# acids-ircam/RAVE

Hardware: NVIDIA H100
Metric: audio-seconds/s (v2 train step fwd+bwd, 48 kHz) (higher is better)
Workload: dtype bf16

## Files before the change

include/rave_b200.h:

```cpp
#ifndef RAVE_B200_H
#define RAVE_B200_H

#include <stddef.h>
#include <stdint.h>

#ifdef __cplusplus
extern "C" {
#endif

#define RAVE_ACT_NONE 0
#define RAVE_ACT_LEAKY 1
#define RAVE_ACT_SNAKE 2

#define RAVE_PREC_FP32 0
#define RAVE_PREC_BF16 1
#define RAVE_PREC_TF32 2

int rave_b200_version(void);
const char *rave_b200_last_error(void);
unsigned long long rave_b200_launch_count(void);

int rave_pqmf_analysis_fwd(const float *x, const float *taps, float *y, int B, int T, int Lout,
                           int ntaps, int pad_l, int flip_sign, void *stream);
int rave_pqmf_synthesis_fwd(const float *x, const float *w, float *out, int B, int L, int K,
// ... 9 lines not shown
                           const float *alpha, int post_act, float post_slope, const float *post_x,
                           const float *post_alpha, void *stream);
int rave_conv1d_scatter_f32(const float *src, const float *w, const float *bias, const float *res,
                            float *out, int B, int Cs, int Ls, int Cm, int Lo, int K, int stride,
                            int dil, int pad_l, long ws_m, long ws_c, int act, float slope,
                            const float *alpha, int post_act, float post_slope, const float *post_x,
                            const float *post_alpha, void *stream);

size_t rave_conv1d_wgrad_workspace_bytes(int B, int Ca, int Cc, int Lp, int K);
int rave_conv1d_wgrad_f32(const float *P, const float *Q, float *dw, int B, int Ca, int Lp, int Cc,
                          int Lq, int K, int stride, int dil, int pad_l, long os_a, long os_c,
                          int act_p, int act_q, float slope, const float *alpha, void *workspace,
                          void *stream);

int rave_weight_norm_fwd(const float *v, const float *g, float *w, float *norm_out, int C0, int R,
                         void *stream);
int rave_weight_norm_bwd(const float *dw, const float *v, const float *g, const float *norm,
                         float *dv, float *dg, int C0, int R, void *stream);

int rave_act_fwd(const float *x, float *y, int B, int C, int L, int act, float slope,
                 const float *alpha, void *stream);
int rave_act_bwd(const float *dy, const float *x, float *dx, float *dalpha, int B, int C, int L,
                 int act, float slope, const float *alpha, void *stream);
int rave_am_tanh_fwd(const float *x, float *y, int B, int C, int L, void *stream);
int rave_am_tanh_bwd(const float *dy, const float *x, float *dx, int B, int C, int L, void *stream);
int rave_reparam_fwd(const float *z, const float *eps, float *zs, float *kl_sum, int B, int C, int L, void *stream);

int rave_conv1d_tc_supported(int Cin, int Cout, int K, int stride, int dil);
int rave_dilated_unit_tc_supported(int C, int L);
int rave_dilated_unit_tc_fwd(const void *xa_bf16, const void *w3t_bf16, const void *w1t_bf16, void *a1_out,
                             float *out_f32, void *out_act, int B, int C, int L, int pitch, int dil, int pad_l,
                             float slope_in, float slope_mid, int act_out, float slope_out, void *stream);
int rave_conv1d_tc_plan(int B, int Cin, int Cout, int Lout, int K);
int rave_conv1d_tc_fwd(const void *xa_bf16, const void *wt_bf16, const float *bias, const float *res,
                       const void *res_bf16, const void *dact_src_bf16, const void *res_act_bf16, float res_slope,
                       float *out_f32, void *out_act_bf16,
                       int B, int Cin, int Lin, int in_pitch, int Cout, int Lout,
                       int K, int stride, int dil, int pad_l, int act, float slope, int out_rows,
                       int out_row_stride, int out_row_offset, const float *fm_d, int fm_bh, void *stream);
int rave_conv1d_tc_fwd_x3(const void *xa_bf16, const void *wt_bf16, const float *bias, const float *res,
                          const void *res_act, float res_slope, float *out_f32, void *out_act, int B, int Cin, int Lin,
                          int in_pitch, int Cout, int Lout, int K, int stride, int dil, int pad_l, int act, float slope,
                          int out_rows, int out_row_stride, int out_row_offset, int act_cs, void *stream);
int rave_conv1d_tc_wgrad_splits(int B, int Cm, int Lp, int Cn, int K);
int rave_time_stack_cl(const float *x, void *out_bf16, int B, int C, int T, int F, int Fp, int Cp, int kt, int pt,
                       void *stream);
int rave_time_stack_cl_bwd(const void *g_bf16, float *gx, int B, int C, int T, int F, int Fp, int Cp, int kt, int pt,
                           void *stream);
int rave_time_stack_nhwc(const float *x, void *out_bf16, int B, int C, int T, int F, long sb, long st, int Fp, int Cp, int kt,
                         int pt, void *stream);
int rave_time_stack_nhwc_bwd(const void *g_bf16, float *gx, int B, int C, int T, int F, int Fp, int Cp, int kt, int pt,
                             void *stream);
int rave_time_stack_nhwc_dil(const float *x, void *out_bf16, int B, int C, int T, int F, long sb, long st, int Fp, int Cp,
                             int kt, int pt, int dil, void *stream);
int rave_time_stack_nhwc_dil_bwd(const void *g_bf16, float *gx, int B, int C, int T, int F, int Fp, int Cp, int kt, int pt,
                                 int dil, void *stream);
int rave_l1_stats_f32(const float *t, const float *v, float *stats, long n, void *stream);
int rave_l1_grad_f32(const float *t, const float *v, const float *d, float *gt, float *gv, long n, void *stream);
int rave_leaky_fm_fwd(const float *x, float *a, float *stats, long H, float slope, void *stream);
int rave_leaky_fm_bwd(const float *a, const float *g, const float *d, float *gx, long H, float slope, void *stream);
int rave_leaky_fm_stack_fwd(const float *x, float *a, float *stats, void *xs_bf16, long Rh, int T, int F, int C, int Fp,
                            float slope, void *stream);
int rave_leaky_fm_stack_bwd(const float *a, const void *gxs_bf16, const float *ga, const float *d, float *gx, long Rh, int T,
                            int F, int C, int Fp, float slope, void *stream);
int rave_leaky_fm_stack_dil_fwd(const float *x, float *a, float *stats, void *xs_bf16, long Rh, int T, int F, int C, int Fp,
                                int dil, float slope, void *stream);
// ... 99 lines not shown
```

rave_b200/_lib.py:

```python
import ctypes
import os
from ctypes import c_float, c_int, c_long, c_size_t, c_ulonglong, c_void_p, c_char_p

_HERE = os.path.dirname(os.path.abspath(__file__))
LIB_PATH = os.path.join(_HERE, "csrc", "librave_b200.so")

_P, _I, _F, _L = c_void_p, c_int, c_float, c_long

SIGNATURES = {
    "rave_b200_version": (c_int, []),
    "rave_b200_last_error": (c_char_p, []),
    "rave_b200_launch_count": (c_ulonglong, []),
    "rave_pqmf_analysis_fwd": (c_int, [_P, _P, _P, _I, _I, _I, _I, _I, _I, _P]),
    "rave_pqmf_synthesis_fwd": (c_int, [_P, _P, _P, _I, _I, _I, _I, _F, _I, _P]),
    "rave_pqmf_analysis_fast": (c_int, [_P, _P, _P, _P, _I, _I, _I, _I, _I, _P]),
    "rave_pqmf_synthesis_fast": (c_int, [_P, _P, _P, _P, _I, _I, _I, _F, _I, _P]),
    "rave_conv1d_gather_f32": (c_int, [_P, _P, _P, _P, _P, _I, _I, _I, _I, _I, _I, _I, _I, _I, _L, _L,
                                       _I, _F, _P, _I, _F, _P, _P, _P]),
    "rave_conv1d_scatter_f32": (c_int, [_P, _P, _P, _P, _P, _I, _I, _I, _I, _I, _I, _I, _I, _I, _L, _L,
                                        _I, _F, _P, _I, _F, _P, _P, _P]),
    "rave_conv1d_wgrad_workspace_bytes": (c_size_t, [_I, _I, _I, _I, _I]),
    "rave_conv1d_wgrad_f32": (c_int, [_P, _P, _P, _I, _I, _I, _I, _I, _I, _I, _I, _I, _L, _L, _I, _I,
                                      _F, _P, _P, _P]),
    "rave_weight_norm_fwd": (c_int, [_P, _P, _P, _P, _I, _I, _P]),
    "rave_weight_norm_bwd": (c_int, [_P, _P, _P, _P, _P, _P, _I, _I, _P]),
    "rave_act_fwd": (c_int, [_P, _P, _I, _I, _I, _I, _F, _P, _P]),
    "rave_act_bwd": (c_int, [_P, _P, _P, _P, _I, _I, _I, _I, _F, _P, _P]),
    "rave_am_tanh_fwd": (c_int, [_P, _P, _I, _I, _I, _P]),
    "rave_am_tanh_bwd": (c_int, [_P, _P, _P, _I, _I, _I, _P]),
    "rave_reparam_fwd": (c_int, [_P, _P, _P, _P, _I, _I, _I, _P]),
    "rave_conv1d_tc_supported": (c_int, [_I, _I, _I, _I, _I]),
    "rave_dilated_unit_tc_supported": (c_int, [_I, _I]),
    "rave_dilated_unit_tc_fwd": (c_int, [_P, _P, _P, _P, _P, _P, _I, _I, _I, _I, _I, _I, _F, _F, _I, _F, _P]),
    "rave_conv1d_tc_plan": (c_int, [_I, _I, _I, _I, _I]),
    "rave_conv1d_tc_fwd": (c_int, [_P, _P, _P, _P, _P, _P, _P, _F, _P, _P, _I, _I, _I, _I, _I, _I, _I, _I, _I, _I, _I,
                                   _F, _I, _I, _I, _P, _I, _P]),
    "rave_conv1d_tc_fwd_x3": (c_int, [_P, _P, _P, _P, _P, _F, _P, _P, _I, _I, _I, _I, _I, _I, _I, _I, _I, _I, _I, _F, _I,
                                      _I, _I, _I, _P]),
    "rave_weight_prep_tc_multi_x3": (c_int, [_I, _P, _P]),
    "rave_ncl_to_cl_x3": (c_int, [_P, _P, _I, _I, _I, _P]),
    "rave_conv1d_tc_wgrad": (c_int, [_P, _P, _P, _P, _I, _I, _I, _I, _I, _I, _I, _I, _I, _I, _I, _P]),
    "rave_tapmajor_to_weight_f32": (c_int, [_P, _P, _I, _I, _I, _I, _I, _P]),
    "rave_conv1d_tc_wgrad_splits": (c_int, [_I, _I, _I, _I, _I]),
    "rave_time_stack_cl": (c_int, [_P, _P, _I, _I, _I, _I, _I, _I, _I, _I, _P]),
    "rave_time_stack_cl_bwd": (c_int, [_P, _P, _I, _I, _I, _I, _I, _I, _I, _I, _P]),
    "rave_time_stack_nhwc": (c_int, [_P, _P, _I, _I, _I, _I, ctypes.c_long, ctypes.c_long, _I, _I, _I, _I, _P]),
    "rave_time_stack_nhwc_bwd": (c_int, [_P, _P, _I, _I, _I, _I, _I, _I, _I, _I, _P]),
    "rave_time_stack_nhwc_dil": (c_int, [_P, _P, _I, _I, _I, _I, ctypes.c_long, ctypes.c_long, _I, _I, _I, _I, _I, _P]),
    "rave_time_stack_nhwc_dil_bwd": (c_int, [_P, _P, _I, _I, _I, _I, _I, _I, _I, _I, _I, _P]),
    "rave_l1_stats_f32": (c_int, [_P, _P, _P, ctypes.c_long, _P]),
    "rave_leaky_fm_fwd": (c_int, [_P, _P, _P, ctypes.c_long, ctypes.c_float, _P]),
    "rave_leaky_fm_bwd": (c_int, [_P, _P, _P, _P, ctypes.c_long, ctypes.c_float, _P]),
    "rave_leaky_fm_stack_fwd": (c_int, [_P, _P, _P, _P, ctypes.c_long, _I, _I, _I, _I, ctypes.c_float, _P]),
    "rave_leaky_fm_stack_bwd": (c_int, [_P, _P, _P, _P, _P, ctypes.c_long, _I, _I, _I, _I, ctypes.c_float, _P]),
    "rave_leaky_fm_stack_dil_fwd": (c_int, [_P, _P, _P, _P, ctypes.c_long, _I, _I, _I, _I, _I, ctypes.c_float, _P]),
    "rave_leaky_fm_stack_dil_bwd": (c_int, [_P, _P, _P, _P, _P, ctypes.c_long, _I, _I, _I, _I, _I, ctypes.c_float, _P]),
    "rave_l1_grad_f32": (c_int, [_P, _P, _P, _P, _P, ctypes.c_long, _P]),
    "rave_snake_cl_fwd": (c_int, [_P, _P, _P, ctypes.c_long, _I, _P]),
    "rave_snake_cl_bwd": (c_int, [_P, _P, _P, _P, _P, _P, ctypes.c_long, _I, _P]),
    "rave_weight_prep_tc": (c_int, [_P, _P, _P, _P, _P, _I, _P, _P, _I, _I, _I, _I, _I, _I, _P]),
    "rave_weight_norm_bwd_tapmajor": (c_int, [_P, _P, _P, _P, _P, _P, _I, _I, _I, _I, _I, _I, _P]),
    "rave_conv1d_c1_fwd": (c_int, [_P, _P, _P, _P, _P, _I, _I, _I, _I, _I, _I, _I, _I, _I, _I, _F, _P]),
    "rave_conv1d_c1_wgrad_splits": (c_int, [_I, _I]),
    "rave_conv1d_c1_wgrad": (c_int, [_P, _P, _P, _I, _I, _I, _I, _I, _I, _I, _I, _I, _I, _P]),
    "rave_conv1d_c1_dgrad": (c_int, [_P, _P, _P, _I, _I, _I, _I, _I, _I, _I, _I, _I, _I, _P]),
    "rave_colsum_bf16": (c_int, [_P, _P, _I, _I, _I, _I, _I, _P]),
    "rave_im2col_c1": (c_int, [_P, _P, _I, _I, _I, _I, _I, _I, _I, _I, _I, _I, _I, _P]),
# ... 109 lines not shown
```

rave_b200/csrc/conv_tc.cu:

```cuda
#include <string.h>

#include "common.cuh"
#include "tc_common.cuh"

namespace rave {
namespace tc {

constexpr int BLOCK_M = 128;
constexpr int NUM_THREADS = 288;
constexpr int SMEM_MAX = 227 * 1024;

struct TcParams {
  int B, Cin, Lin, Cout, Lout, K, stride, dil, pad_l;
  int BL, BB;
  int n_lt, n_bg, n_nt;
  int num_kb;
  int act;
  float slope;
  const float *bias;
  const float *res;
  const __nv_bfloat16 *res_bf16;
  const __nv_bfloat16 *dact_src;
  const __nv_bfloat16 *res_act;
  float res_inv_slope;
  float *out_f32;
  __nv_bfloat16 *out_act;
  int out_rows;
  int out_row_stride;
  int out_row_offset;
  const float *fm_d;
  long fm_half;
  int fm_bh;
  int x3;
  int act_ld;
  int act_cs;
  int stages, nacc;
  int stg;
  int acc_off, stg_off, bar_off;
};

template <int BLOCK_N, int BLOCK_K, bool X3 = false>
struct SmemLayout {
  static constexpr int PARTS = X3 ? 2 : 1;
  static constexpr int A_PART = BLOCK_M * BLOCK_K * 2;
  static constexpr int B_PART = (BLOCK_N * BLOCK_K * 2 + 1023) / 1024 * 1024;
  static constexpr int A_BYTES = PARTS * A_PART;
  static constexpr int B_BYTES = PARTS * BLOCK_N * BLOCK_K * 2;
  static constexpr int B_BYTES_PAD = PARTS * B_PART;
  static constexpr int STAGE_BYTES = A_BYTES + B_BYTES_PAD;
  static constexpr int ACC_LD = acc_pitch(BLOCK_N);
  static constexpr int ACC_BYTES = BLOCK_M * ACC_LD * 4;
  static constexpr int OUT_BOXC = BLOCK_N % 64 == 0 ? 64 : BLOCK_N % 32 == 0 ? 32 : 16;
  static constexpr int OUT_SPAN = OUT_BOXC * 2;
  static constexpr int STG_BYTES = X3 ? 0 : BLOCK_M * BLOCK_N * 2;
  static constexpr int FIXED = 256 + 1024;
  static constexpr int stages_for(int nacc, int stg) {
    const int s = (SMEM_MAX - FIXED - nacc * ACC_BYTES - stg * STG_BYTES) / STAGE_BYTES;
    return s > 8 ? 8 : s;
  }
};

template <int BLOCK_N, int BLOCK_K, bool X3>
static void plan_smem(int kblocks, TcParams &p) {
  using L = SmemLayout<BLOCK_N, BLOCK_K, X3>;
  const int base = L::stages_for(1, 0);
  const int need = kblocks + 1 < base ? kblocks + 1 : base;
  p.nacc = 1;
  p.stg = 0;
  if (L::stages_for(2, 1) >= need) { p.nacc = 2; p.stg = 1; }
  else if (L::stages_for(1, 1) >= need) p.stg = 1;
  if (X3) p.stg = 0;
// ... 289 lines not shown
      const int bg = mt / p.n_lt;
      const int n0 = nt * BLOCK_N;
      const int b = bg * p.BB + row / p.BL;
      const int l = lt * p.BL + row % p.BL;
      const bool valid = (b < p.B) && (l < p.Lout);
      const size_t orow = (size_t)b * p.out_rows + (size_t)l * p.out_row_stride + p.out_row_offset;

      const int buf = p.nacc == 2 ? (it & 1) : 0;
      const uint32_t use = p.nacc == 2 ? (it >> 1) : it;
      if (stg) {
        if (issuer) bulk_wait_read<0>();
        named_bar_sync(1, 128);
      }
      mbar_wait(&tfull_bar[buf], use & 1);
      const uint32_t taddr = (uint32_t)(128 * buf + quad * 32) << 16;
      tc_epilogue<BLOCK_N, X3, BOXC>(p, taddr, n0, valid, orow, p.fm_d ? (b < p.fm_bh ? 1 : -1) : 0, stg, row);
      __syncwarp();
      if (lane == 0) mbar_arrive(&tempty_bar[buf]);
      if (stg) {
        fence_proxy_async();
        named_bar_sync(1, 128);
        if (issuer) {
#pragma unroll
          for (int c = 0; c < BLOCK_N; c += BOXC)
            tma_store_3d(&tmap_o, stg + (c / BOXC) * (BLOCK_M * L::OUT_SPAN), n0 + c, lt * p.BL, bg * p.BB);
          bulk_commit();
        }
      }
    }
    if (stg && issuer) bulk_wait_all();
  }
}

typedef CUresult (*EncodeTiledFn)(CUtensorMap *, CUtensorMapDataType, cuuint32_t, void *, const cuuint64_t *,
                                  const cuuint64_t *, const cuuint32_t *, const cuuint32_t *,
                                  CUtensorMapInterleave, CUtensorMapSwizzle, CUtensorMapL2promotion,
                                  CUtensorMapFloatOOBfill);

static EncodeTiledFn get_encode_fn() {
  static EncodeTiledFn fn = nullptr;
  if (!fn) {
    void *ptr = nullptr;
    cudaDriverEntryPointQueryResult q;
    if (cudaGetDriverEntryPoint("cuTensorMapEncodeTiled", &ptr, cudaEnableDefault, &q) == cudaSuccess &&
        q == cudaDriverEntryPointSuccess)
      fn = (EncodeTiledFn)ptr;
  }
  return fn;
}

static CUtensorMapSwizzle swizzle_enum(int bytes) {
  return bytes == 128 ? CU_TENSOR_MAP_SWIZZLE_128B : bytes == 64 ? CU_TENSOR_MAP_SWIZZLE_64B
                                                                 : CU_TENSOR_MAP_SWIZZLE_32B;
}

static int pick_block_k(int Cin) {
  if (Cin % 64 == 0) return 64;
  if (Cin % 32 == 0) return 32;
  if (Cin % 16 == 0) return 16;
  return 0;
}

static int pick_block_n(int Cout, long m_tiles) {
  const int cands[] = {128, 96, 64, 48, 32, 16};
  constexpr int NC = sizeof(cands) / sizeof(cands[0]);
  int best = 0;
  for (int c : cands) {
    if (Cout % c) continue;
    if (!best) best = c;
    if (m_tiles * (Cout / c) >= 132) return c;
  }
  for (int i = NC - 1; i >= 0; --i)
    if (Cout % cands[i] == 0 && cands[i] >= 32) return cands[i];
  return best;
}

template <int BN, int BK, bool X3>
static int launch(const CUtensorMap &ta, const CUtensorMap &tb, TcParams p, cudaStream_t stream) {
  using L = SmemLayout<BN, BK, X3>;
  plan_smem<BN, BK, X3>(p.K * p.num_kb, p);
  if (!p.out_act) p.stg = 0;
  const int smem = p.bar_off + L::FIXED;
  static int attr = 0;
  if (smem > attr) {
    cudaError_t e = cudaFuncSetAttribute(conv_tc_kernel<BN, BK, X3>, cudaFuncAttributeMaxDynamicSharedMemorySize, smem);
    if (e != cudaSuccess) {
      set_error("conv1d_tc: cudaFuncSetAttribute(%d bytes): %s", smem, cudaGetErrorString(e));
      return 2;
    }
    attr = smem;
  }
  CUtensorMap to;
  memset(&to, 0, sizeof(to));
  if (p.stg) {
    EncodeTiledFn enc = get_encode_fn();
    cuuint64_t dims[3] = {(cuuint64_t)p.Cout, (cuuint64_t)p.Lout, (cuuint64_t)p.B};
    cuuint64_t strides[2] = {(cuuint64_t)p.Cout * 2 * p.out_row_stride, (cuuint64_t)p.Cout * 2 * p.out_rows};
    cuuint32_t box[3] = {(cuuint32_t)L::OUT_BOXC, (cuuint32_t)p.BL, (cuuint32_t)p.BB};
    cuuint32_t estr[3] = {1, 1, 1};
    CUresult r = enc(&to, CU_TENSOR_MAP_DATA_TYPE_BFLOAT16, 3, p.out_act + (size_t)p.out_row_offset * p.Cout, dims,
                     strides, box, estr, CU_TENSOR_MAP_INTERLEAVE_NONE, swizzle_enum(L::OUT_SPAN),
                     CU_TENSOR_MAP_L2_PROMOTION_NONE, CU_TENSOR_MAP_FLOAT_OOB_FILL_NONE);
    if (r != CUDA_SUCCESS) {
      set_error("conv1d_tc: output tensor map encode failed (%d)", (int)r);
      return 1;
    }
  }
  const int tiles = p.n_lt * p.n_bg * p.n_nt;
  int dev = 0, sms = 132;
  cudaGetDevice(&dev);
  cudaDeviceGetAttribute(&sms, cudaDevAttrMultiProcessorCount, dev);
  const int grid = tiles < sms ? tiles : sms;
  launch_pdl(conv_tc_kernel<BN, BK, X3>, dim3(grid), dim3(NUM_THREADS), smem, stream, ta, tb, to, p);
  RAVE_CHECK_LAUNCH("conv1d_tc");
  return 0;
}

template <int BK, bool X3>
static int dispatch_n(int bn, const CUtensorMap &ta, const CUtensorMap &tb, const TcParams &p,
                      cudaStream_t s) {
  switch (bn) {
    case 128: return launch<128, BK, X3>(ta, tb, p, s);
    case 96: return launch<96, BK, X3>(ta, tb, p, s);
    case 64: return launch<64, BK, X3>(ta, tb, p, s);
    case 48: return launch<48, BK, X3>(ta, tb, p, s);
    case 32: return launch<32, BK, X3>(ta, tb, p, s);
    case 16: return launch<16, BK, X3>(ta, tb, p, s);
  }
  set_error("conv1d_tc: no kernel for BLOCK_N=%d", bn);
  return 1;
}

template <int BK>
static int smem_plan_bits(int BN, int kblocks) {
  TcParams q;
  switch (BN) {
    case 128: plan_smem<128, BK, false>(kblocks, q); break;
    case 96: plan_smem<96, BK, false>(kblocks, q); break;
    case 64: plan_smem<64, BK, false>(kblocks, q); break;
    case 48: plan_smem<48, BK, false>(kblocks, q); break;
// ... 17 lines not shown

int conv_tc_dispatch_x3(int BK, int BN, const CUtensorMap &ta, const CUtensorMap &tb, const TcParams &p, cudaStream_t s);
#ifdef RAVE_TC_X3_UNIT
int conv_tc_dispatch_x3(int BK, int BN, const CUtensorMap &ta, const CUtensorMap &tb, const TcParams &p, cudaStream_t s) {
  return dispatch_all<true>(BK, BN, ta, tb, p, s);
}
#endif

}
}

#ifndef RAVE_TC_X3_UNIT
extern "C" int rave_conv1d_tc_supported(int Cin, int Cout, int K, int stride, int dil) {
  if (rave::tc::pick_block_k(Cin) == 0) return 0;
  if (Cout % 16) return 0;
  if (K < 1 || stride < 1 || dil < 1) return 0;
  return 1;
}

extern "C" int rave_conv1d_tc_plan(int B, int Cin, int Cout, int Lout, int K) {
  using namespace rave;
  using namespace rave::tc;
  const int BK = pick_block_k(Cin);
  if (!BK || Cout % 16) return 0;
  int BL = 128;
  while (BL > Lout && BL > 8) BL >>= 1;
  const long m_tiles = (long)ceil_div(Lout, BL) * ceil_div(B, 128 / BL);
  const int BN = pick_block_n(Cout, m_tiles);
  if (!BN) return 0;
  const int kblocks = K * ceil_div(Cin, BK);
  const int smem = BK == 64 ? smem_plan_bits<64>(BN, kblocks)
                 : BK == 32 ? smem_plan_bits<32>(BN, kblocks) : smem_plan_bits<16>(BN, kblocks);
  return BN | (BK << 12) | smem;
}

static int conv1d_tc_fwd_impl(const void *xa, const void *wt, const float *bias, const float *res,
                              const void *res_bf16, const void *dact_src, const void *res_act, float res_slope,
                              float *out_f32, void *out_act,
                              int B, int Cin, int Lin, int in_pitch, int Cout, int Lout,
                              int K, int stride, int dil, int pad_l, int act, float slope, int out_rows,
                              int out_row_stride, int out_row_offset, const float *fm_d, int fm_bh,
                              void *stream, int x3, int act_cs = 0) {
  using namespace rave;
  using namespace rave::tc;
  RAVE_CHECK_ARG(!x3 || (!res_bf16 && !dact_src && !fm_d),
                 "conv1d_tc(x3): the split-operand mode has no gradient epilogues (forward path only)");
  RAVE_CHECK_ARG(xa && wt && (out_f32 || out_act), "conv1d_tc: null pointer");
  RAVE_CHECK_ARG(rave_conv1d_tc_supported(Cin, Cout, K, stride, dil), "conv1d_tc: unsupported shape Cin=%d Cout=%d",
                 Cin, Cout);
  if (in_pitch <= 0) in_pitch = Lin;
  RAVE_CHECK_ARG(in_pitch >= ceil_div(Lin, stride) * stride,
                 "conv1d_tc: input pitch %d < Lin %d rounded up to the stride %d (slack rows must be zero)", in_pitch,
                 Lin, stride);
  RAVE_CHECK_ARG(act == RAVE_ACT_NONE || act == RAVE_ACT_LEAKY, "conv1d_tc: epilogue activation %d unsupported", act);
  RAVE_CHECK_ARG(act != RAVE_ACT_LEAKY || (slope >= 0.f && slope <= 1.f), "conv1d_tc: LeakyReLU slope %g outside [0, 1]",
                 (double)slope);
  RAVE_CHECK_ARG(!res_act || (res_slope > 0.f && res_slope <= 1.f), "conv1d_tc: res_slope %g outside (0, 1]",
                 (double)res_slope);
  RAVE_CHECK_ARG(((uintptr_t)bias & 15) == 0, "conv1d_tc: bias must be 16-byte aligned");
  RAVE_CHECK_ARG(((uintptr_t)xa & 15) == 0 && ((uintptr_t)wt & 15) == 0, "conv1d_tc: operands must be 16B aligned");
  RAVE_CHECK_ARG((((uintptr_t)out_f32 | (uintptr_t)out_act | (uintptr_t)res | (uintptr_t)res_bf16 | (uintptr_t)dact_src |
                   (uintptr_t)res_act) & 31) == 0,
                 "conv1d_tc: epilogue tensors must be 32-byte aligned (256-bit row segments)");
  EncodeTiledFn enc = get_encode_fn();
  RAVE_CHECK_ARG(enc, "conv1d_tc: cuTensorMapEncodeTiled not available");

// ... 26 lines not shown
  while (BL > Lout && BL > 8) BL >>= 1;
  p.BL = BL; p.BB = 128 / BL;
  p.n_lt = ceil_div(Lout, BL);
  p.n_bg = ceil_div(B, p.BB);
  const int BN = pick_block_n(Cout, (long)p.n_lt * p.n_bg);
  RAVE_CHECK_ARG(BN > 0, "conv1d_tc: no BLOCK_N for Cout=%d", Cout);
  p.n_nt = Cout / BN;
  p.num_kb = ceil_div(Cin, BK);

  CUtensorMap ta, tb;
  {
    const cuuint64_t ca = (cuuint64_t)Cin * (x3 ? 2 : 1);
    cuuint64_t dims[4] = {ca, (cuuint64_t)stride, (cuuint64_t)ceil_div(Lin, stride), (cuuint64_t)B};
    cuuint64_t strides[3] = {ca * 2, ca * 2 * stride, ca * 2 * in_pitch};
    cuuint32_t box[4] = {(cuuint32_t)BK, 1, (cuuint32_t)p.BL, (cuuint32_t)p.BB};
    cuuint32_t estr[4] = {1, 1, 1, 1};
    CUresult r = enc(&ta, CU_TENSOR_MAP_DATA_TYPE_BFLOAT16, 4, const_cast<void *>(xa), dims, strides, box, estr,
                     CU_TENSOR_MAP_INTERLEAVE_NONE, swizzle_enum(BK * 2), promo,
                     CU_TENSOR_MAP_FLOAT_OOB_FILL_NONE);
    RAVE_CHECK_ARG(r == CUDA_SUCCESS, "conv1d_tc: tensor map A encode failed (%d)", (int)r);
  }
  {
    cuuint64_t dims[2] = {(cuuint64_t)Cin, (cuuint64_t)K * Cout * (x3 ? 2 : 1)};
    cuuint64_t strides[1] = {(cuuint64_t)Cin * 2};
    cuuint32_t box[2] = {(cuuint32_t)BK, (cuuint32_t)BN};
    cuuint32_t estr[2] = {1, 1};
    CUresult r = enc(&tb, CU_TENSOR_MAP_DATA_TYPE_BFLOAT16, 2, const_cast<void *>(wt), dims, strides, box, estr,
                     CU_TENSOR_MAP_INTERLEAVE_NONE, swizzle_enum(BK * 2), promo,
                     CU_TENSOR_MAP_FLOAT_OOB_FILL_NONE);
    RAVE_CHECK_ARG(r == CUDA_SUCCESS, "conv1d_tc: tensor map B encode failed (%d)", (int)r);
  }
  cudaStream_t s = (cudaStream_t)stream;
  if (x3) return conv_tc_dispatch_x3(BK, BN, ta, tb, p, s);
  return dispatch_all<false>(BK, BN, ta, tb, p, s);
}

extern "C" int rave_conv1d_tc_fwd(const void *xa, const void *wt, const float *bias, const float *res,
                                  const void *res_bf16, const void *dact_src, const void *res_act, float res_slope,
                                  float *out_f32, void *out_act,
                                  int B, int Cin, int Lin, int in_pitch, int Cout, int Lout,
                                  int K, int stride, int dil, int pad_l, int act, float slope, int out_rows,
                                  int out_row_stride, int out_row_offset, const float *fm_d, int fm_bh,
                                  void *stream) {
  return conv1d_tc_fwd_impl(xa, wt, bias, res, res_bf16, dact_src, res_act, res_slope, out_f32, out_act, B, Cin, Lin,
                            in_pitch, Cout, Lout, K, stride, dil, pad_l, act, slope, out_rows, out_row_stride,
                            out_row_offset, fm_d, fm_bh, stream, 0);
}

extern "C" int rave_conv1d_tc_fwd_x3(const void *xa, const void *wt, const float *bias, const float *res,
                                     const void *res_act, float res_slope, float *out_f32, void *out_act,
                                     int B, int Cin, int Lin, int in_pitch, int Cout, int Lout,
                                     int K, int stride, int dil, int pad_l, int act, float slope, int out_rows,
                                     int out_row_stride, int out_row_offset, int act_cs, void *stream) {
  return conv1d_tc_fwd_impl(xa, wt, bias, res, nullptr, nullptr, res_act, res_slope, out_f32, out_act, B, Cin, Lin,
                            in_pitch, Cout, Lout, K, stride, dil, pad_l, act, slope, out_rows, out_row_stride,
                            out_row_offset, nullptr, 0, stream, 1, act_cs);
}

namespace rave {
namespace tc {

constexpr int WG_ROWS = 64;
constexpr int WG_SLAB = WG_ROWS * 128;

struct WgParams {
  int B, Cm, Lp, Cn, Lq, K, stride, dil, pad_l;
// ... 320 lines not shown
```

rave_b200/csrc/tc_common.cuh:

```cuda
#pragma once
#include <cuda.h>
#include <cuda_runtime.h>
#include <stdint.h>
#include <string.h>

#include "wgmma_sm90.cuh"

namespace rave {
namespace tc {

__device__ __forceinline__ uint32_t smem_u32(const void *p) {
  return (uint32_t)__cvta_generic_to_shared(p);
}

__device__ __forceinline__ void mbar_init(uint64_t *bar, uint32_t count) {
  asm volatile("mbarrier.init.shared::cta.b64 [%0], %1;" ::"r"(smem_u32(bar)), "r"(count));
}
__device__ __forceinline__ void fence_barrier_init() {
  asm volatile("fence.mbarrier_init.release.cluster;" ::: "memory");
}
__device__ __forceinline__ void fence_proxy_async() {
  asm volatile("fence.proxy.async.shared::cta;" ::: "memory");
}
__device__ __forceinline__ void mbar_arrive_expect_tx(uint64_t *bar, uint32_t bytes) {
// ... 84 lines not shown
}
__device__ __forceinline__ void tma_store_3d(const CUtensorMap *m, const void *smem, int c0, int c1, int c2) {
  asm volatile("cp.async.bulk.tensor.3d.global.shared::cta.bulk_group [%0, {%2, %3, %4}], [%1];" ::"l"(m),
               "r"(smem_u32(smem)), "r"(c0), "r"(c1), "r"(c2)
               : "memory");
}
__device__ __forceinline__ void tma_store_4d(const CUtensorMap *m, const void *smem, int c0, int c1, int c2, int c3) {
  asm volatile("cp.async.bulk.tensor.4d.global.shared::cta.bulk_group [%0, {%2, %3, %4, %5}], [%1];" ::"l"(m),
               "r"(smem_u32(smem)), "r"(c0), "r"(c1), "r"(c2), "r"(c3)
               : "memory");
}
__device__ __forceinline__ void bulk_commit() { asm volatile("cp.async.bulk.commit_group;" ::: "memory"); }
template <int N>
__device__ __forceinline__ void bulk_wait_read() {
  asm volatile("cp.async.bulk.wait_group.read %0;" ::"n"(N) : "memory");
}
__device__ __forceinline__ void bulk_wait_all() { asm volatile("cp.async.bulk.wait_group 0;" ::: "memory"); }
__device__ __forceinline__ void named_bar_sync(int id, int threads) {
  asm volatile("bar.sync %0, %1;" ::"r"(id), "r"(threads) : "memory");
}
__device__ __forceinline__ void lds128(const void *p, uint32_t *r) {
  asm volatile("ld.shared.v4.b32 {%0,%1,%2,%3}, [%4];" : "=r"(r[0]), "=r"(r[1]), "=r"(r[2]), "=r"(r[3])
               : "r"(smem_u32(p)));
}
__device__ __forceinline__ void sts128(void *p, const uint32_t *r) {
  asm volatile("st.shared.v4.b32 [%0], {%1,%2,%3,%4};" ::"r"(smem_u32(p)), "r"(r[0]), "r"(r[1]), "r"(r[2]), "r"(r[3])
               : "memory");
}

__device__ __forceinline__ void wgmma_fence() { asm volatile("wgmma.fence.sync.aligned;" ::: "memory"); }
__device__ __forceinline__ void wgmma_commit() { asm volatile("wgmma.commit_group.sync.aligned;" ::: "memory"); }
template <int N>
__device__ __forceinline__ void wgmma_wait() { asm volatile("wgmma.wait_group.sync.aligned %0;" ::"n"(N) : "memory"); }
template <int R>
__device__ __forceinline__ void wgmma_fence_regs(float *d) {
#pragma unroll
  for (int i = 0; i < R; ++i) asm volatile("" : "+f"(d[i])::"memory");
}

static __shared__ uint32_t s_acc_addr, s_acc_ld;
__host__ __device__ constexpr int acc_pitch(int cols) { return (cols + 31) / 32 * 32 + 4; }
__device__ __forceinline__ void acc_bind(const void *buf, int ld) {
  s_acc_addr = smem_u32(buf);
  s_acc_ld = (uint32_t)ld;
}
template <int N>
__device__ __forceinline__ void acc_store(const float (*d)[N / 2], int wg_thread, int col0 = 0, int row0 = 0) {
  const int w = wg_thread >> 5, l = wg_thread & 31;
  const uint32_t ld = s_acc_ld;
#pragma unroll
  for (int h = 0; h < 2; ++h) {
    const uint32_t r0 = (uint32_t)(row0 + 64 * h + 16 * w + (l >> 2));
#pragma unroll
    for (int j = 0; j < N / 8; ++j) {
      const uint32_t c = (uint32_t)(col0 + 8 * j + 2 * (l & 3));
      const uint32_t a0 = s_acc_addr + (r0 * ld + c) * 4u, a1 = a0 + 8u * ld * 4u;
      asm volatile("st.shared.v2.f32 [%0], {%1, %2};" ::"r"(a0), "f"(d[h][4 * j]), "f"(d[h][4 * j + 1]) : "memory");
      asm volatile("st.shared.v2.f32 [%0], {%1, %2};" ::"r"(a1), "f"(d[h][4 * j + 2]), "f"(d[h][4 * j + 3]) : "memory");
    }
  }
}
template <int NC>
__device__ __forceinline__ void acc_ld(uint32_t taddr, float *v) {
  const uint32_t row = (taddr >> 16) + (threadIdx.x & 31), col = taddr & 0xFFFFu;
  const uint32_t a = s_acc_addr + (row * s_acc_ld + col) * 4u;
#pragma unroll
// ... 87 lines not shown
```

Baseline: 2013.

## Add ping-pong warp-specialized conv kernel for backward activation-grad epilogue path

Adds a persistent 3-warpgroup conv kernel: one producer warp issues TMA loads for A/B stages plus the epilogue operands (activation mask, feature-match partner, bf16 residual) into double-buffered slots, while two consumer warpgroups alternate tiles with ordered mainloops so one group's epilogue overlaps the other's wgmma. Register budgets are rebalanced with setmaxnreg and the output is written back with TMA stores. It is dispatched only for the bf16 no-bias, no-activation case that has a dact source; other cases keep the old kernel. The operand slots take shared memory, which lowers the number of pipeline stages.

```diff
diff --git a/include/rave_b200.h b/include/rave_b200.h
--- a/include/rave_b200.h
+++ b/include/rave_b200.h
@@ -65,6 +65,7 @@
                              float *out_f32, void *out_act, int B, int C, int L, int pitch, int dil, int pad_l,
                              float slope_in, float slope_mid, int act_out, float slope_out, void *stream);
 int rave_conv1d_tc_plan(int B, int Cin, int Cout, int Lout, int K);
+int rave_conv1d_tc_pp_stages(int B, int Cin, int Cout, int Lout, int K, int fm, int res_bf16);
 int rave_conv1d_tc_fwd(const void *xa_bf16, const void *wt_bf16, const float *bias, const float *res,
                        const void *res_bf16, const void *dact_src_bf16, const void *res_act_bf16, float res_slope,
                        float *out_f32, void *out_act_bf16,
diff --git a/rave_b200/_lib.py b/rave_b200/_lib.py
--- a/rave_b200/_lib.py
+++ b/rave_b200/_lib.py
@@ -33,6 +33,7 @@
     "rave_dilated_unit_tc_supported": (c_int, [_I, _I]),
     "rave_dilated_unit_tc_fwd": (c_int, [_P, _P, _P, _P, _P, _P, _I, _I, _I, _I, _I, _I, _F, _F, _I, _F, _P]),
     "rave_conv1d_tc_plan": (c_int, [_I, _I, _I, _I, _I]),
+    "rave_conv1d_tc_pp_stages": (c_int, [_I, _I, _I, _I, _I, _I, _I]),
     "rave_conv1d_tc_fwd": (c_int, [_P, _P, _P, _P, _P, _P, _P, _F, _P, _P, _I, _I, _I, _I, _I, _I, _I, _I, _I, _I, _I,
                                    _F, _I, _I, _I, _P, _I, _P]),
     "rave_conv1d_tc_fwd_x3": (c_int, [_P, _P, _P, _P, _P, _F, _P, _P, _I, _I, _I, _I, _I, _I, _I, _I, _I, _I, _I, _F, _I,
diff --git a/rave_b200/csrc/conv_tc.cu b/rave_b200/csrc/conv_tc.cu
--- a/rave_b200/csrc/conv_tc.cu
+++ b/rave_b200/csrc/conv_tc.cu
@@ -37,6 +37,7 @@
   int stages, nacc;
   int stg;
   int acc_off, stg_off, bar_off;
+  int ops_off, ops_bytes;
 };
 
 template <int BLOCK_N, int BLOCK_K, bool X3 = false>
@@ -392,6 +393,230 @@
   }
 }
 
+constexpr int PP_THREADS = 384;
+
+template <int BLOCK_N, int BOXC, bool FM, bool RS>
+__device__ __forceinline__ void pp_epilogue(float (*d)[BLOCK_N / 2], uint8_t *slot, const TcParams &p, int w, int lane,
+                                            int b0) {
+  constexpr int TILE_BYTES = BLOCK_M * BLOCK_N * 2;
+  uint8_t *part = slot + TILE_BYTES;
+  uint8_t *skip = slot + (FM ? 2 : 1) * TILE_BYTES;
+  constexpr int SPAN = BOXC * 2, JB = BOXC / 8;
+  const float d0 = FM ? __ldg(p.fm_d) : 0.f, d1 = FM ? __ldg(p.fm_d + 1) : 0.f;
+  const uint32_t base = stg_offset<BOXC>(16 * w + (lane >> 2), 0) + 4 * (lane & 3);
+#pragma unroll
+  for (int h = 0; h < 2; ++h) {
+#pragma unroll
+    for (int r = 0; r < 2; ++r) {
+      const int row = 64 * h + 16 * w + (lane >> 2) + 8 * r;
+      const float d1r = (FM && b0 + row / p.BL < p.fm_bh) ? d1 : 0.f;
+#pragma unroll
+      for (int j = 0; j < BLOCK_N / 8; ++j) {
+        const uint32_t off = (base ^ (uint32_t)((j % JB) << 4)) + (j / JB) * (BLOCK_M * SPAN) + (64 * h + 8 * r) * SPAN;
+        float v0 = d[h][4 * j + 2 * r], v1 = d[h][4 * j + 2 * r + 1];
+        const uint32_t dm = *reinterpret_cast<const uint32_t *>(slot + off);
+        if (dm & 0x00008000u) v0 *= p.slope;
+        if (dm & 0x80000000u) v1 *= p.slope;
+        if (FM) {
+          const uint32_t pm = *reinterpret_cast<const uint32_t *>(part + off);
+#pragma unroll
+          for (int e = 0; e < 2; ++e) {
+            const float as = e ? bf_hi(dm) : bf_lo(dm);
+            const float ap = e ? bf_hi(pm) : bf_lo(pm);
+            const float t = (as > ap ? 1.f : 0.f) - (as < ap ? 1.f : 0.f);
+            const float sr = (as > 0.f ? 1.f : 0.f) - (as < 0.f ? 1.f : 0.f);
+            float &v = e ? v1 : v0;
+            v = fmaf(d1r, sr, fmaf(d0, t, v));
+          }
+        }
+        if (RS) {
+          const uint32_t rb = *reinterpret_cast<const uint32_t *>(skip + off);
+          v0 += bf_lo(rb);
+          v1 += bf_hi(rb);
+        }
+        __nv_bfloat162 o = __floats2bfloat162_rn(v0, v1);
+        *reinterpret_cast<uint32_t *>(slot + off) = *reinterpret_cast<uint32_t *>(&o);
+      }
+    }
+  }
+}
+
+template <int BLOCK_N, int BLOCK_K, bool FM, bool RS>
+__global__ void __launch_bounds__(PP_THREADS, 1)
+conv_tc_pp_kernel(const __grid_constant__ CUtensorMap tmap_a, const __grid_constant__ CUtensorMap tmap_b,
+                  const __grid_constant__ CUtensorMap tmap_m, const __grid_constant__ CUtensorMap tmap_p,
+                  const __grid_constant__ CUtensorMap tmap_r, const __grid_constant__ CUtensorMap tmap_o,
+                  const TcParams p) {
+  using L = SmemLayout<BLOCK_N, BLOCK_K, false>;
+  constexpr int BOXC = L::OUT_BOXC;
+  constexpr int BOX_BYTES = BLOCK_M * L::OUT_SPAN;
+  constexpr int TILE_BYTES = BLOCK_M * BLOCK_N * 2;
+  constexpr int SWZ = BLOCK_K * 2;
+  const int STAGES = p.stages;
+  static_assert(BLOCK_N % 16 == 0 && BLOCK_N >= 16 && BLOCK_N <= 128, "invalid wgmma N");
+
+  extern __shared__ uint8_t smem_raw[];
+  uint8_t *smem = reinterpret_cast<uint8_t *>((reinterpret_cast<uintptr_t>(smem_raw) + 1023) & ~uintptr_t(1023));
+  uint64_t *full_bar = reinterpret_cast<uint64_t *>(smem + p.bar_off);
+  uint64_t *empty_bar = full_bar + STAGES;
+  uint64_t *ofull_bar = empty_bar + STAGES;
+  uint64_t *oempty_bar = ofull_bar + 2;
+  uint64_t *order_bar = oempty_bar + 2;
+
+  const int wg = threadIdx.x >> 7;
+  const int warp = threadIdx.x >> 5;
+  const int lane = threadIdx.x & 31;
+  const int num_tiles = p.n_lt * p.n_bg * p.n_nt;
+  const int kblocks = p.K * p.num_kb;
+  constexpr bool fm = FM, rs = RS;
+
+  if (threadIdx.x == 0) {
+    tma_prefetch_desc(&tmap_a);
+    tma_prefetch_desc(&tmap_b);
+    tma_prefetch_desc(&tmap_m);
+    tma_prefetch_desc(&tmap_o);
+    if (fm) tma_prefetch_desc(&tmap_p);
+    if (rs) tma_prefetch_desc(&tmap_r);
+    for (int s = 0; s < STAGES; ++s) {
+      mbar_init(&full_bar[s], 1);
+      mbar_init(&empty_bar[s], 4);
+    }
+    for (int c = 0; c < 2; ++c) {
+      mbar_init(&ofull_bar[c], 1);
+      mbar_init(&oempty_bar[c], 1);
+      mbar_init(&order_bar[c], 4);
+    }
+    fence_barrier_init();
+  }
+  __syncthreads();
+  griddep_launch_dependents();
+  griddep_wait();
+
+  if (wg == 0) {
+    warpgroup_reg_dealloc<56>();
+    if (warp != 0) return;
+    int stage = 0;
+    uint32_t phase = 0;
+    int it = 0;
+    for (int tile = blockIdx.x; tile < num_tiles; tile += gridDim.x, ++it) {
+      const int nt = tile % p.n_nt;
+      const int mt = tile / p.n_nt;
+      const int lt = mt % p.n_lt;
+      const int bg = mt / p.n_lt;
+      const int l0 = lt * p.BL;
+      const int b0 = bg * p.BB;
+      const int n0 = nt * BLOCK_N;
+      const int c = it & 1;
+      for (int k = 0; k < p.K; ++k) {
+        const int off = k * p.dil - p.pad_l;
+        int j = off / p.stride;
+        int ph = off - j * p.stride;
+        if (ph < 0) { ph += p.stride; j -= 1; }
+        for (int kb = 0; kb < p.num_kb; ++kb) {
+          mbar_wait(&empty_bar[stage], phase ^ 1);
+          uint8_t *sa = smem + stage * L::STAGE_BYTES;
+          uint8_t *sb = sa + L::A_BYTES;
+          if (elect_one()) {
+            mbar_arrive_expect_tx(&full_bar[stage], L::A_BYTES + L::B_BYTES);
+            tma_load_4d(sa, &tmap_a, &full_bar[stage], kb * BLOCK_K, ph, l0 + j, b0);
+            tma_load_2d(sb, &tmap_b, &full_bar[stage], kb * BLOCK_K, k * p.Cout + n0);
+          }
+          __syncwarp();
+          if (++stage == STAGES) { stage = 0; phase ^= 1; }
+          if (k == 0 && kb == 0) {
+            mbar_wait(&oempty_bar[c], ((it >> 1) & 1) ^ 1);
+            uint8_t *slot = smem + p.ops_off + c * p.ops_bytes;
+            if (elect_one()) {
+              mbar_arrive_expect_tx(&ofull_bar[c], p.ops_bytes);
+              for (int cb = 0; cb < BLOCK_N / BOXC; ++cb) {
+                tma_load_3d(slot + cb * BOX_BYTES, &tmap_m, &ofull_bar[c], n0 + cb * BOXC, l0, b0);
+                if (fm) {
+                  for (int i = 0; i < p.BB; ++i) {
+                    const int b = b0 + i;
+                    const int pb = p.fm_bh > 0 ? (b < p.fm_bh ? b + p.fm_bh : b - p.fm_bh) : b;
+                    tma_load_3d(slot + TILE_BYTES + cb * BOX_BYTES + i * p.BL * L::OUT_SPAN, &tmap_p, &ofull_bar[c],
+                                n0 + cb * BOXC, l0, pb);
+                  }
+                }
+                if (rs)
+                  tma_load_3d(slot + (fm ? 2 : 1) * TILE_BYTES + cb * BOX_BYTES, &tmap_r, &ofull_bar[c], n0 + cb * BOXC,
+                              l0, b0);
+              }
+            }
+            __syncwarp();
+          }
+        }
+      }
+    }
+  } else {
+    warpgroup_reg_alloc<224>();
+    const int c = wg - 1;
+    const int w = warp & 3;
+    const bool issuer = (threadIdx.x & 127) == 0;
+    constexpr uint64_t A_HALF = (64 * SWZ) >> 4;
+    const uint32_t smem_base = smem_u32(smem);
+    uint8_t *slot = smem + p.ops_off + c * p.ops_bytes;
+    float d[2][BLOCK_N / 2];
+    int u = 0;
+    for (int tile = blockIdx.x + c * gridDim.x; tile < num_tiles; tile += 2 * gridDim.x, ++u) {
+      const int it = 2 * u + c;
+      const uint32_t g0 = (uint32_t)it * (uint32_t)kblocks;
+      int stage = (int)(g0 % (uint32_t)STAGES);
+      uint32_t phase = (g0 / (uint32_t)STAGES) & 1;
+      if (it > 0) mbar_wait(&order_bar[c], ((it - 1) >> 1) & 1);
+      int prev = 0;
+      for (int kb = 0; kb < kblocks; ++kb) {
+        mbar_wait(&full_bar[stage], phase);
+        const uint32_t sa = smem_base + stage * L::STAGE_BYTES;
+        const uint64_t adesc = make_kmajor_desc(sa, SWZ);
+        const uint64_t bdesc = make_kmajor_desc(sa + L::A_BYTES, SWZ);
+        wgmma_fence();
+#pragma unroll
+        for (int kk = 0; kk < BLOCK_K / 16; ++kk) {
+#pragma unroll
+          for (int h = 0; h < 2; ++h)
+            Wgmma<BLOCK_N, 0, 0>::mma(d[h], adesc + h * A_HALF + 2 * kk, bdesc + 2 * kk, (kb > 0 || kk > 0) ? 1u : 0u);
+        }
+        wgmma_commit();
+        wgmma_wait<1>();
+        if (kb > 0) {
+          __syncwarp();
+          if (lane == 0) mbar_arrive(&empty_bar[prev]);
+        }
+        prev = stage;
+        if (++stage == STAGES) { stage = 0; phase ^= 1; }
+      }
+      __syncwarp();
+      if (lane == 0) mbar_arrive(&order_bar[c ^ 1]);
+      wgmma_wait<0>();
+      wgmma_fence_regs<BLOCK_N / 2>(d[0]);
+      wgmma_fence_regs<BLOCK_N / 2>(d[1]);
+      __syncwarp();
+      if (lane == 0) mbar_arrive(&empty_bar[prev]);
+
+      const int nt = tile % p.n_nt;
+      const int mt = tile / p.n_nt;
+      const int lt = mt % p.n_lt;
+      const int bg = mt / p.n_lt;
+      const int b0 = bg * p.BB;
+      const int n0 = nt * BLOCK_N;
+      mbar_wait(&ofull_bar[c], u & 1);
+      pp_epilogue<BLOCK_N, BOXC, FM, RS>(d, slot, p, w, lane, b0);
+      fence_proxy_async();
+      named_bar_sync(1 + c, 128);
+      if (issuer) {
+#pragma unroll
+        for (int cb = 0; cb < BLOCK_N / BOXC; ++cb)
+          tma_store_3d(&tmap_o, slot + cb * BOX_BYTES, n0 + cb * BOXC, lt * p.BL, b0);
+        bulk_commit();
+        bulk_wait_read<0>();
+        mbar_arrive(&oempty_bar[c]);
+      }
+    }
+    if (issuer) bulk_wait_all();
+  }
+}
+
 typedef CUresult (*EncodeTiledFn)(CUtensorMap *, CUtensorMapDataType, cuuint32_t, void *, const cuuint64_t *,
                                   const cuuint64_t *, const cuuint32_t *, const cuuint32_t *,
                                   CUtensorMapInterleave, CUtensorMapSwizzle, CUtensorMapL2promotion,
@@ -434,6 +659,112 @@
     if (Cout % cands[i] == 0 && cands[i] >= 32) return cands[i];
   return best;
 }
+
+template <int BN>
+static int encode_rows_map(CUtensorMap *m, const __nv_bfloat16 *base, const TcParams &p, int box_b) {
+  using L = SmemLayout<BN, 64, false>;
+  EncodeTiledFn enc = get_encode_fn();
+  cuuint64_t dims[3] = {(cuuint64_t)p.Cout, (cuuint64_t)p.Lout, (cuuint64_t)p.B};
+  cuuint64_t strides[2] = {(cuuint64_t)p.Cout * 2 * p.out_row_stride, (cuuint64_t)p.Cout * 2 * p.out_rows};
+  cuuint32_t box[3] = {(cuuint32_t)L::OUT_BOXC, (cuuint32_t)p.BL, (cuuint32_t)box_b};
+  cuuint32_t estr[3] = {1, 1, 1};
+  CUresult r = enc(m, CU_TENSOR_MAP_DATA_TYPE_BFLOAT16, 3, const_cast<__nv_bfloat16 *>(base) + (size_t)p.out_row_offset * p.Cout,
+                   dims, strides, box, estr, CU_TENSOR_MAP_INTERLEAVE_NONE, swizzle_enum(L::OUT_SPAN),
+                   CU_TENSOR_MAP_L2_PROMOTION_NONE, CU_TENSOR_MAP_FLOAT_OOB_FILL_NONE);
+  if (r != CUDA_SUCCESS) {
+    set_error("conv1d_tc: bf16 row tensor map encode failed (%d)", (int)r);
+    return 1;
+  }
+  return 0;
+}
+
+template <int BLOCK_N, int BLOCK_K>
+static bool plan_smem_pp(int nops, TcParams &p) {
+  using L = SmemLayout<BLOCK_N, BLOCK_K, false>;
+  p.ops_bytes = nops * BLOCK_M * BLOCK_N * 2;
+  const int s = (SMEM_MAX - L::FIXED - 2 * p.ops_bytes) / L::STAGE_BYTES;
+  p.stages = s > 8 ? 8 : s;
+  p.ops_off = p.stages * L::STAGE_BYTES;
+  p.bar_off = p.ops_off + 2 * p.ops_bytes;
+  return p.stages >= 2;
+}
+
+template <int BN, int BK>
+static int launch_pp(const CUtensorMap &ta, const CUtensorMap &tb, TcParams p, cudaStream_t stream) {
+  using L = SmemLayout<BN, BK, false>;
+  if (!plan_smem_pp<BN, BK>(1 + (p.fm_d ? 1 : 0) + (p.res_bf16 ? 1 : 0), p)) return -1;
+  const int smem = p.bar_off + L::FIXED;
+  const int v = (p.fm_d ? 2 : 0) + (p.res_bf16 ? 1 : 0);
+  void (*kern)(CUtensorMap, CUtensorMap, CUtensorMap, CUtensorMap, CUtensorMap, CUtensorMap, TcParams) =
+      v == 3 ? conv_tc_pp_kernel<BN, BK, true, true> : v == 2 ? conv_tc_pp_kernel<BN, BK, true, false>
+      : v == 1 ? conv_tc_pp_kernel<BN, BK, false, true> : conv_tc_pp_kernel<BN, BK, false, false>;
+  static int attr[4] = {0, 0, 0, 0};
+  if (smem > attr[v]) {
+    cudaError_t e = cudaFuncSetAttribute(kern, cudaFuncAttributeMaxDynamicSharedMemorySize, smem);
+    if (e != cudaSuccess) {
+      set_error("conv1d_tc: cudaFuncSetAttribute(%d bytes): %s", smem, cudaGetErrorString(e));
+      return 1;
+    }
+    attr[v] = smem;
+  }
+  CUtensorMap tm, tp, tr, to;
+  memset(&tp, 0, sizeof(tp));
+  memset(&tr, 0, sizeof(tr));
+  if (encode_rows_map<BN>(&tm, p.dact_src, p, p.BB) || encode_rows_map<BN>(&to, p.out_act, p, p.BB)) return 1;
+  if (p.fm_d && encode_rows_map<BN>(&tp, p.fm_bh > 0 ? p.dact_src : p.dact_src - p.fm_half, p, 1)) return 1;
+  if (p.res_bf16 && encode_rows_map<BN>(&tr, p.res_bf16, p, p.BB)) return 1;
+  const int tiles = p.n_lt * p.n_bg * p.n_nt;
+  int dev = 0, sms = 132;
+  cudaGetDevice(&dev);
+  cudaDeviceGetAttribute(&sms, cudaDevAttrMultiProcessorCount, dev);
+  const int grid = tiles < sms ? tiles : sms;
+  launch_pdl(kern, dim3(grid), dim3(PP_THREADS), smem, stream, ta, tb, tm, tp, tr, to, p);
+  RAVE_CHECK_LAUNCH("conv1d_tc");
+  return 0;
+}
+
+#ifndef RAVE_TC_X3_UNIT
+template <int BK>
+static int dispatch_pp_n(int bn, const CUtensorMap &ta, const CUtensorMap &tb, const TcParams &p, cudaStream_t s) {
+  switch (bn) {
+    case 128: return launch_pp<128, BK>(ta, tb, p, s);
+    case 96:
+      if constexpr (BK == 64) return -1;
+      else return launch_pp<96, BK>(ta, tb, p, s);
+    case 64: return launch_pp<64, BK>(ta, tb, p, s);
+    case 48: return launch_pp<48, BK>(ta, tb, p, s);
+    case 32: return launch_pp<32, BK>(ta, tb, p, s);
+    case 16: return launch_pp<16, BK>(ta, tb, p, s);
+  }
+  set_error("conv1d_tc: no kernel for BLOCK_N=%d", bn);
+  return 1;
+}
+
+static int dispatch_pp(int BK, int BN, const CUtensorMap &ta, const CUtensorMap &tb, const TcParams &p, cudaStream_t s) {
+  switch (BK) {
+    case 64: return dispatch_pp_n<64>(BN, ta, tb, p, s);
+    case 32: return dispatch_pp_n<32>(BN, ta, tb, p, s);
+    case 16: return dispatch_pp_n<16>(BN, ta, tb, p, s);
+  }
+  set_error("conv1d_tc: no kernel for BLOCK_K=%d", BK);
+  return 1;
+}
+
+template <int BK>
+static int pp_stages(int BN, int nops) {
+  TcParams q;
+  bool ok = false;
+  switch (BN) {
+    case 128: ok = plan_smem_pp<128, BK>(nops, q); break;
+    case 96: ok = BK != 64 && plan_smem_pp<96, BK>(nops, q); break;
+    case 64: ok = plan_smem_pp<64, BK>(nops, q); break;
+    case 48: ok = plan_smem_pp<48, BK>(nops, q); break;
+    case 32: ok = plan_smem_pp<32, BK>(nops, q); break;
+    case 16: ok = plan_smem_pp<16, BK>(nops, q); break;
+  }
+  return ok ? q.stages : 0;
+}
+#endif
 
 template <int BN, int BK, bool X3>
 static int launch(const CUtensorMap &ta, const CUtensorMap &tb, TcParams p, cudaStream_t stream) {
@@ -452,20 +783,7 @@
   }
   CUtensorMap to;
   memset(&to, 0, sizeof(to));
-  if (p.stg) {
-    EncodeTiledFn enc = get_encode_fn();
-    cuuint64_t dims[3] = {(cuuint64_t)p.Cout, (cuuint64_t)p.Lout, (cuuint64_t)p.B};
-    cuuint64_t strides[2] = {(cuuint64_t)p.Cout * 2 * p.out_row_stride, (cuuint64_t)p.Cout * 2 * p.out_rows};
-    cuuint32_t box[3] = {(cuuint32_t)L::OUT_BOXC, (cuuint32_t)p.BL, (cuuint32_t)p.BB};
-    cuuint32_t estr[3] = {1, 1, 1};
-    CUresult r = enc(&to, CU_TENSOR_MAP_DATA_TYPE_BFLOAT16, 3, p.out_act + (size_t)p.out_row_offset * p.Cout, dims,
-                     strides, box, estr, CU_TENSOR_MAP_INTERLEAVE_NONE, swizzle_enum(L::OUT_SPAN),
-                     CU_TENSOR_MAP_L2_PROMOTION_NONE, CU_TENSOR_MAP_FLOAT_OOB_FILL_NONE);
-    if (r != CUDA_SUCCESS) {
-      set_error("conv1d_tc: output tensor map encode failed (%d)", (int)r);
-      return 1;
-    }
-  }
+  if (p.stg && encode_rows_map<BN>(&to, p.out_act, p, p.BB)) return 1;
   const int tiles = p.n_lt * p.n_bg * p.n_nt;
   int dev = 0, sms = 132;
   cudaGetDevice(&dev);
@@ -549,6 +867,14 @@
   const int smem = BK == 64 ? smem_plan_bits<64>(BN, kblocks)
                  : BK == 32 ? smem_plan_bits<32>(BN, kblocks) : smem_plan_bits<16>(BN, kblocks);
   return BN | (BK << 12) | smem;
+}
+
+extern "C" int rave_conv1d_tc_pp_stages(int B, int Cin, int Cout, int Lout, int K, int fm, int res_bf16) {
+  using namespace rave::tc;
+  const int plan = rave_conv1d_tc_plan(B, Cin, Cout, Lout, K);
+  const int BN = plan & 0xFFF, BK = (plan >> 12) & 0xFFF;
+  const int nops = 1 + (fm ? 1 : 0) + (res_bf16 ? 1 : 0);
+  return BK == 64 ? pp_stages<64>(BN, nops) : BK == 32 ? pp_stages<32>(BN, nops) : BK == 16 ? pp_stages<16>(BN, nops) : 0;
 }
 
 static int conv1d_tc_fwd_impl(const void *xa, const void *wt, const float *bias, const float *res,
@@ -641,6 +967,10 @@
   }
   cudaStream_t s = (cudaStream_t)stream;
   if (x3) return conv_tc_dispatch_x3(BK, BN, ta, tb, p, s);
+  if (dact_src && out_act && !bias && !res && !res_act && !out_f32 && act == RAVE_ACT_NONE) {
+    const int r = dispatch_pp(BK, BN, ta, tb, p, s);
+    if (r >= 0) return r;
+  }
   return dispatch_all<false>(BK, BN, ta, tb, p, s);
 }
 
diff --git a/rave_b200/csrc/tc_common.cuh b/rave_b200/csrc/tc_common.cuh
--- a/rave_b200/csrc/tc_common.cuh
+++ b/rave_b200/csrc/tc_common.cuh
@@ -140,6 +140,14 @@
 __device__ __forceinline__ void wgmma_commit() { asm volatile("wgmma.commit_group.sync.aligned;" ::: "memory"); }
 template <int N>
 __device__ __forceinline__ void wgmma_wait() { asm volatile("wgmma.wait_group.sync.aligned %0;" ::"n"(N) : "memory"); }
+template <int N>
+__device__ __forceinline__ void warpgroup_reg_dealloc() {
+  asm volatile("setmaxnreg.dec.sync.aligned.u32 %0;" ::"n"(N));
+}
+template <int N>
+__device__ __forceinline__ void warpgroup_reg_alloc() {
+  asm volatile("setmaxnreg.inc.sync.aligned.u32 %0;" ::"n"(N));
+}
 template <int R>
 __device__ __forceinline__ void wgmma_fence_regs(float *d) {
 #pragma unroll
```

New measurement: 2173, median of 6. 7.9% higher.
